# jiahuei/sparse-image-captioning

Measured on AMD Instinct MI355X. Metric: captions/sec, higher is better.
Workload: dtype bf16; 1 GPU; configs[1]: ORT dense, 256 images x 5 captions, teacher-forcing XE fwd+bwd+clip+Adam; images_per_gpu=256, regions=36, captions_per_image=5, parallelism=single

## Files before the change

### include/ortk.h

```cpp
#ifndef ORTK_H
#define ORTK_H

#include <stddef.h>
#include <stdint.h>

#ifdef __cplusplus
extern "C" {
#endif

#define ORTK_VERSION 19
#define ORTK_EINVAL (-1)
#define ORTK_ENOSPC (-2)
#define ORTK_ENOSYS (-3)
#define ORTK_EEXCHANGE (-4)

typedef void* ortk_stream;

int ortk_version(void);
int ortk_device_ok(void);

struct ortk_sparse_plan;
typedef struct ortk_config {
    int32_t d_model, d_ff, n_layers, n_heads;
    int32_t vocab, feat, seq_len;
    int32_t pad_id, bos_id, eos_id, unk_id;
    int32_t box_trig;
    int32_t precision;
    float   drop_src, drop;
    int32_t share_enc[16], share_dec[16];
    int32_t share_att_enc, share_att_dec;
    int32_t no_box;
    const struct ortk_sparse_plan* sparse_fwd;
    const struct ortk_sparse_plan* sparse_bwd;
// ... 120 lines not shown
int ortk_row_bchain(const ortk_bchain_args* a, ortk_stream stream);
int ortk_row_bchain_plan(const ortk_bchain_args* a, int32_t* rows_per_block, int32_t* workgroups);

typedef struct ortk_tuning {
    int32_t gemm_t64;
    int32_t attn_impl;
    int32_t attn16_min_lq;
    int32_t side_stream;
    int32_t row_chain;
    int32_t chain_wide;
    int32_t spmm_alias;
    int32_t f32_split;
    int32_t wgrad_wgs;
    int32_t wgrad_group;
    int32_t wgrad_group_splitk;
    int32_t wgrad_group_wgs;
    int32_t wgrad_group_tail;
    int32_t feats_bf16;
    int32_t ln_fuse;
    int32_t samp_epilogue;
    int32_t gemm_epilogue;
    int32_t attn16_short;
    int32_t attn16_block;
} ortk_tuning;
void ortk_get_tuning(ortk_tuning* out);
int ortk_set_tuning(const ortk_tuning* t);

#define ORTK_DEC_UNFUSED 1
#define ORTK_DEC_STACK 2
#define ORTK_DEC_SPARSE_STREAM 4
#define ORTK_DEC_STACK_RB20 8
#define ORTK_DEC_STACK_SPLIT 16
#define ORTK_DEC_SPLIT_SMALL 32
#define ORTK_DEC_SPARSE_GATHER 64
#define ORTK_DEC_STACK_FP8 128
#define ORTK_DEC_GROUPS_JOINT 65536
#define ORTK_MAX_BEAM 32
typedef struct ortk_decode_opts {
    int32_t beam_size;
    int32_t num_random_sample;
    float   temperature;
    int32_t decoding_constraint;
    int32_t length_penalty;
    double  length_alpha;
    uint64_t seed;
    const struct ortk_sparse_plan* sparse;
// ... 29 lines not shown


typedef struct ortk_gemm_args {
    const void* A; const void* B; void* C;
    int64_t lda, ldb, ldc;
    int32_t M, N, K, transA, transB;
    const float* bias; const float* rowscale; const float* resid; int64_t ldr;
    const void* gate; int64_t ldg; float gate_scale;
    int32_t relu; float drop_p; uint32_t drop_seed;
    int32_t accumulate, splitk, precision;
    int32_t a_dtype, b_dtype, c_dtype, gate_dtype;
    float* colsum;
    int32_t drop_row_stride, drop_row_off;
    int32_t ln_mode, ln_y_dtype;
    const float* ln_a; const float* ln_b; void* ln_y; float* ln_stats; float ln_eps;
    const float* ln_x; const float* ln_dres; float* ln_da; float* ln_db;
    float* tile_stats; int32_t stat_ncols;
    const int32_t* drop_rows;
    float* tile_samp; const int64_t* samp_seq; uint64_t samp_seed; int64_t samp_row_offset;
    int32_t samp_L, samp_t, samp_greedy_stride, samp_sample, samp_fast, samp_no_store; float samp_inv_temperature;
} ortk_gemm_args;
int ortk_gemm(const ortk_gemm_args* a, ortk_stream stream);
int ortk_gemm_plan(const ortk_gemm_args* a, char* buf, int32_t buf_bytes);
#define ORTK_WGRAD_MAX 8
typedef struct ortk_wgrad_item {
    const void* dY; int64_t lddy;
    const void* X; int64_t ldx;
    float* dW; int64_t lddw;
    float* db;
    int32_t Nout, Kin;
} ortk_wgrad_item;
typedef struct ortk_wgrad_group_args {
    ortk_wgrad_item item[ORTK_WGRAD_MAX];
    int32_t n, splitk;
    int64_t rows;
    int32_t flags;
    void* ws; size_t ws_bytes;
} ortk_wgrad_group_args;
int ortk_wgrad_group(const ortk_wgrad_group_args* a, ortk_stream stream);
size_t ortk_wgrad_group_workspace_bytes(const ortk_wgrad_group_args* a);
int ortk_prof_enable(int32_t on);
int ortk_prof_collect(int32_t key, int64_t* launches, double* total_ms, double* total_flops);
int ortk_prof_collect_bytes(int32_t key, double* total_bytes);
int ortk_prof_collect_units(int32_t key, double* total_workgroups);

int ortk_layernorm_fwd(const float* x, const float* a, const float* b, void* y, int32_t y_dtype, float* stats,
// ... 141 lines not shown
```

### sparse-image-captioning_amd/_lib.py

```python
import ctypes as C
import os

import torch

_HERE = os.path.dirname(os.path.abspath(__file__))
LIB_PATH = os.path.join(_HERE, "libortk.so")


class OrtkUnavailable(RuntimeError):
    pass


class OrtkError(RuntimeError):
    pass


class Config(C.Structure):
    _fields_ = [("d_model", C.c_int32), ("d_ff", C.c_int32), ("n_layers", C.c_int32), ("n_heads", C.c_int32),
                ("vocab", C.c_int32), ("feat", C.c_int32), ("seq_len", C.c_int32),
                ("pad_id", C.c_int32), ("bos_id", C.c_int32), ("eos_id", C.c_int32), ("unk_id", C.c_int32),
                ("box_trig", C.c_int32), ("precision", C.c_int32), ("drop_src", C.c_float), ("drop", C.c_float),
                ("share_enc", C.c_int32 * 16), ("share_dec", C.c_int32 * 16),
                ("share_att_enc", C.c_int32), ("share_att_dec", C.c_int32), ("no_box", C.c_int32),
                ("sparse_fwd", C.c_void_p), ("sparse_bwd", C.c_void_p)]
# ... 60 lines not shown
class MaskedAdamArgs(C.Structure):
    _fields_ = [("w", C.c_void_p), ("g", C.c_void_p), ("mw", C.c_void_p), ("vw", C.c_void_p),
                ("ml", C.c_void_p), ("mm", C.c_void_p), ("mv", C.c_void_p),
                ("draws", C.c_void_p), ("active", C.c_void_p), ("extra_coef", C.c_void_p),
                ("n", C.c_int64), ("index0", C.c_int64), ("mode", C.c_int32), ("seed", C.c_uint32),
                ("lr_w", C.c_float), ("eps_w", C.c_float), ("lr_m", C.c_float), ("eps_m", C.c_float),
                ("beta1", C.c_float), ("beta2", C.c_float), ("clip", C.c_float), ("bc1", C.c_float), ("bc2", C.c_float)]


OPT_ADAM, OPT_SGD, OPT_SGDM, OPT_SGDMOM, OPT_RMSPROP, OPT_ADAGRAD = range(6)
OPT_KINDS = {"adam": OPT_ADAM, "sgd": OPT_SGD, "sgdm": OPT_SGDM, "sgdmom": OPT_SGDMOM, "rmsprop": OPT_RMSPROP, "adagrad": OPT_ADAGRAD}


class OptimArgs(C.Structure):
    _fields_ = [("p", C.c_void_p), ("g", C.c_void_p), ("s1", C.c_void_p), ("s2", C.c_void_p), ("n", C.c_int64),
                ("kind", C.c_int32), ("first_step", C.c_int32), ("zero_grad", C.c_int32),
                ("lr", C.c_float), ("weight_decay", C.c_float), ("alpha", C.c_float), ("beta", C.c_float), ("eps", C.c_float),
                ("clip", C.c_float), ("bc1", C.c_float), ("bc2", C.c_float)]


class Tuning(C.Structure):
    _fields_ = [("gemm_t64", C.c_int32), ("attn_impl", C.c_int32), ("attn16_min_lq", C.c_int32),
                ("side_stream", C.c_int32), ("row_chain", C.c_int32), ("chain_wide", C.c_int32), ("spmm_alias", C.c_int32), ("f32_split", C.c_int32), ("wgrad_wgs", C.c_int32),
                ("wgrad_group", C.c_int32), ("wgrad_group_splitk", C.c_int32), ("wgrad_group_wgs", C.c_int32), ("wgrad_group_tail", C.c_int32), ("feats_bf16", C.c_int32), ("ln_fuse", C.c_int32), ("samp_epilogue", C.c_int32), ("gemm_epilogue", C.c_int32), ("attn16_short", C.c_int32), ("attn16_block", C.c_int32)]


class LnSlot(C.Structure):
    _fields_ = [("part", C.c_void_p), ("nblocks", C.c_int32), ("da", C.c_void_p), ("db", C.c_void_p)]


MAX_BEAM = 32
DEC_UNFUSED, DEC_STACK, DEC_SPARSE_STREAM, DEC_STACK_RB20, DEC_STACK_SPLIT, DEC_SPLIT_SMALL, DEC_SPARSE_GATHER, DEC_STACK_FP8 = 1, 2, 4, 8, 16, 32, 64, 128
DEC_GROUPS_JOINT = 1 << 16


class DecodeOpts(C.Structure):
    _fields_ = [("beam_size", C.c_int32), ("num_random_sample", C.c_int32), ("temperature", C.c_float),
                ("decoding_constraint", C.c_int32), ("length_penalty", C.c_int32), ("length_alpha", C.c_double),
                ("seed", C.c_uint64), ("sparse", C.POINTER(EllPlanStruct)), ("exec_flags", C.c_int32), ("with_greedy", C.c_int32), ("sample_row_offset", C.c_int64),
                ("train", C.c_int32), ("drop_seed", C.c_uint64), ("memory", C.c_void_p), ("top_k", C.c_int32), ("top_p", C.c_float),
                ("group_size", C.c_int32), ("diversity_lambda", C.c_float)]


class GemmArgs(C.Structure):
    _fields_ = [("A", C.c_void_p), ("B", C.c_void_p), ("C", C.c_void_p),
                ("lda", C.c_int64), ("ldb", C.c_int64), ("ldc", C.c_int64),
                ("M", C.c_int32), ("N", C.c_int32), ("K", C.c_int32), ("transA", C.c_int32), ("transB", C.c_int32),
# ... 57 lines not shown
    "ortk_valid_positions_ok": (_I32, [_CFG, _I32, _I32, _I32, _I32]),
    "ortk_forward": (_I32, [_CFG, _P, C.POINTER(Batch), _P, _SZ, _P, _I64, _I32, _U64, _P]),
    "ortk_forward_phase": (_I32, [_CFG, _P, C.POINTER(Batch), _P, _SZ, _P, _I64, _I32, _U64, _I32, _P]),
    "ortk_train_workspace_memory": (_P, [_CFG, _I32, _I32, _I32, _I32, _P, C.POINTER(C.c_int32)]),
    "ortk_loss": (_I32, [_CFG, C.POINTER(Batch), _P, _SZ, _P, _P, _P]),
    "ortk_loss_smooth": (_I32, [_CFG, C.POINTER(Batch), _P, _SZ, _P, _P, _F, _P]),
    "ortk_loss_external": (_I32, [_CFG, C.POINTER(Batch), _P, _SZ, _P, _P, _I64, _P]),
    "ortk_backward": (_I32, [_CFG, _P, _P, C.POINTER(Batch), _P, _SZ, _I32, _U64, _P]),
    "ortk_backward_phase": (_I32, [_CFG, _P, _P, C.POINTER(Batch), _P, _SZ, _I32, _U64, _I32, _P]),
    "ortk_arena_decoder_offset": (_I64, [_CFG]),
    "ortk_decode_workspace_bytes": (_SZ, [_CFG, _I32, _I32, C.POINTER(DecodeOpts)]),
    "ortk_decode": (_I32, [_CFG, _P, _P, _P, _P, _I32, _I32, C.POINTER(DecodeOpts), _P, _SZ, _P, _P, _P, _P]),
    "ortk_decode_status": (_I32, [_P, _P]),
    "ortk_encode": (_I32, [_CFG, _P, _P, _P, _P, _I32, _I32, _P, _SZ, _P, _P]),
    "ortk_chain_packed_bytes": (_SZ, [_I32]),
    "ortk_row_chain": (_I32, [C.POINTER(ChainArgs), _P]),
    "ortk_row_bchain": (_I32, [C.POINTER(BChainArgs), _P]),
    "ortk_row_chain_plan": (_I32, [C.POINTER(ChainArgs), C.POINTER(_I32), C.POINTER(_I32), C.POINTER(_I32), C.POINTER(_I32)]),
    "ortk_row_bchain_plan": (_I32, [C.POINTER(BChainArgs), C.POINTER(_I32), C.POINTER(_I32)]),
    "ortk_get_tuning": (None, [C.POINTER(Tuning)]),
    "ortk_set_tuning": (_I32, [C.POINTER(Tuning)]),
    "ortk_gemm": (_I32, [C.POINTER(GemmArgs), _P]),
    "ortk_gemm_plan": (_I32, [C.POINTER(GemmArgs), C.c_char_p, _I32]),
    "ortk_wgrad_group": (_I32, [C.POINTER(WgradGroupArgs), _P]),
    "ortk_wgrad_group_workspace_bytes": (_SZ, [C.POINTER(WgradGroupArgs)]),
    "ortk_prof_enable": (_I32, [_I32]),
    "ortk_prof_collect": (_I32, [_I32, C.POINTER(_I64), C.POINTER(C.c_double), C.POINTER(C.c_double)]),
    "ortk_prof_collect_bytes": (_I32, [_I32, C.POINTER(C.c_double)]),
    "ortk_prof_collect_units": (_I32, [_I32, C.POINTER(C.c_double)]),
    "ortk_layernorm_fwd": (_I32, [_P, _P, _P, _P, _I32, _P, _I64, _I32, _F, _P]),
    "ortk_layernorm_bwd": (_I32, [_P, _P, _P, _P, _P, _P, _P, _P, _I64, _I32, _F, _P]),
    "ortk_layernorm_bwd_drop": (_I32, [_P, _P, _P, _P, _P, _P, _P, _P, _I64, _I32, _F, _P, _I32, _F, C.c_uint32, _P]),
    "ortk_layernorm_bwd_drop_rows": (_I32, [_P, _P, _P, _P, _P, _P, _P, _P, _I64, _I32, _F, _P, _I32, _F, C.c_uint32, _P, _P]),
    "ortk_layernorm_bwd_dt": (_I32, [_P, _I32, _P, _P, _P, _P, _P, _P, _P, _I64, _I32, _F, _P, _I32, _F, C.c_uint32, _P, _P]),
    "ortk_layernorm_bwd_part": (_I32, [_P, _I32, _P, _P, _P, _P, _P, _P, _I64, C.POINTER(_I32), _I64, _I32, _F, _P, _I32, _F, C.c_uint32, _P, _P]),
    "ortk_ln_part_blocks": (_I32, [_I64]),
    "ortk_ln_part_rows": (_I32, []),
    "ortk_ln_partials_reduce": (_I32, [C.POINTER(LnSlot), _I32, _P]),
    "ortk_box_logbias_fwd": (_I32, [_P, C.POINTER(_P), C.POINTER(_P), C.POINTER(_F), _P, _I32, _I32, _I32, _I32, _P]),
    "ortk_box_logbias_bwd": (_I32, [_P, C.POINTER(_P), C.POINTER(_P), C.POINTER(_F), _P, C.POINTER(_P), C.POINTER(_P),
                                   _I32, _I32, _I32, _I32, _P]),
    "ortk_box_embedding": (_I32, [_P, C.POINTER(_F), _P, _I32, _I32, _P]),
    "ortk_attention_fwd": (_I32, [C.POINTER(AttnArgs), _P]),
    "ortk_attention_bwd": (_I32, [C.POINTER(AttnArgs), _P]),
    "ortk_attention_plan": (_I32, [C.POINTER(AttnArgs), _I32, C.c_char_p, _I32]),
    "ortk_valid_position_tables": (_I32, [_P, _I32, _I32, _P, _P, _P]),
# ... 20 lines not shown
    "ortk_adam_clip": (_I32, [_P, _P, _P, _P, _I64, _F, _F, _F, _F, _F, _F, _F, _P]),
    "ortk_adam_clip_zero": (_I32, [_P, _P, _P, _P, _I64, _F, _F, _F, _F, _F, _F, _F, _P]),
    "ortk_optim_states": (_I32, [_I32]),
    "ortk_optim_step": (_I32, [C.POINTER(OptimArgs), _P]),
    "ortk_mask_apply": (_I32, [_P, _P, _P, _I64, _I32, _U32, _P]),
    "ortk_mask_bwd": (_I32, [_P, _P, _P, _P, _P, _I64, _I32, _U32, _P, _P]),
    "ortk_masked_adam_step": (_I32, [C.POINTER(MaskedAdamArgs), _P]),
    "ortk_mask_count": (_I32, [_P, _I64, _I32, _P, _P]),
    "ortk_mask_select_workspace_bytes": (_SZ, [_I32, _I32, _I32, _I32]),
    "ortk_mask_select": (_I32, [_P, _P, _P, _P, _P, _P, _P, _P, _P, _I32, _I32, _I32, _I32, _P, _SZ, _P]),
    "ortk_mask_apply_draws": (_I32, [_P, _P, _P, _P, _I64, _P]),
    "ortk_mask_bwd_draws": (_I32, [_P, _P, _P, _P, _P, _P, _I64, _P, _P]),
    "ortk_decode_step_workspace_bytes": (_SZ, [_CFG, _I32]),
    "ortk_project_memory": (_I32, [_CFG, _P, _P, _I64, _P, _SZ, _P, _P]),
    "ortk_decode_step": (_I32, [_CFG, _P, _P, _I32, _I32, _I32, _I32, _P, _P, _P, _P, _I32, _P, _SZ, _P, _I64, _P]),
    "ortk_axpy_cols": (_I32, [_P, _P, _I32, _I64, _I64, _I32, _P]),
    "ortk_linear_block": (_I32, [_CFG, _I32, C.POINTER(C.c_int64), C.POINTER(C.c_int32), C.POINTER(C.c_int32)]),
    "ortk_sparse_build": (_I32, [C.POINTER(EllPlanStruct), _P, _I32, _P]),
    "ortk_spmm": (_I32, [C.POINTER(EllPlanStruct), _I32, C.POINTER(SpmmArgs), _P]),
    "ortk_spmm_plan": (_I32, [C.POINTER(EllPlanStruct), _I32, C.POINTER(SpmmArgs), C.c_char_p, _I32]),
}

_lib = None
ABI_VERSION = 19


def lib():
    global _lib
    if _lib is None:
        if not os.path.exists(LIB_PATH):
            raise OrtkUnavailable(
                f"{LIB_PATH} is missing: build it with `python -c 'import __graft_entry__ as g; g.build()'` "
                "(or `make -C sparse-image-captioning_amd/csrc`).  There is no CPU / PyTorch fallback.")
        h = C.CDLL(LIB_PATH)
        h.ortk_version.restype = C.c_int32
        if h.ortk_version() != ABI_VERSION:
            raise OrtkUnavailable(
                f"{LIB_PATH} is ABI version {h.ortk_version()}, these bindings were written for version {ABI_VERSION} (include/ortk.h: "
                "ORTK_VERSION): a stale build.  Rebuild it with `make -C sparse-image-captioning_amd/csrc`.")
        for name, (res, args) in SIGNATURES.items():
            fn = getattr(h, name)
            fn.restype = res
            fn.argtypes = args
        _lib = h
    return _lib


def set_tuning(**kw):
    t = Tuning()
    lib().ortk_get_tuning(C.byref(t))
    old = {f: getattr(t, f) for f, _ in Tuning._fields_}
    for k, v in kw.items():
        assert k in old, k
        setattr(t, k, int(v))
    check(lib().ortk_set_tuning(C.byref(t)), "ortk_set_tuning")
    return old


def gemm_plan(args):
    buf = C.create_string_buffer(256)
    check(lib().ortk_gemm_plan(C.byref(args), buf, len(buf)), "ortk_gemm_plan")
    return [k for k in buf.value.decode().split(";") if k]


def row_chain_plan(args):
    v = [C.c_int32() for _ in range(4)]
    check(lib().ortk_row_chain_plan(C.byref(args), *[C.byref(x) for x in v]), "ortk_row_chain_plan")
    return dict(zip(("form", "rows_per_block", "workgroups", "prefetchers"), (x.value for x in v)))


def row_bchain_plan(args):
    v = [C.c_int32() for _ in range(2)]
    check(lib().ortk_row_bchain_plan(C.byref(args), *[C.byref(x) for x in v]), "ortk_row_bchain_plan")
    return dict(zip(("rows_per_block", "workgroups"), (x.value for x in v)))


def attention_plan(args, bwd=False):
    buf = C.create_string_buffer(256)
    check(lib().ortk_attention_plan(C.byref(args), int(bool(bwd)), buf, len(buf)), "ortk_attention_plan")
    return [k for k in buf.value.decode().split(";") if k]


def spmm_plan(plan, block, args):
    if hasattr(plan, "ref"):
        plan = plan.ref()
    elif isinstance(plan, EllPlanStruct):
        plan = C.pointer(plan)
# ... 38 lines not shown
```

### sparse-image-captioning_amd/csrc/ortk_gemm.hip

```cpp
#include <algorithm>
#include <cstring>
#include <type_traits>
#include "ortk_internal.h"

namespace {

constexpr int BM = 128, BN = 128;
constexpr int PITCH = 128 + 16;

__device__ __forceinline__ int xcd_remap(int bid, int nwg) {
    const int q = nwg >> 3, r = nwg & 7, x = bid & 7, i = bid >> 3;
    return (x < r ? x * (q + 1) : r * (q + 1) + (x - r) * q) + i;
}

__device__ __forceinline__ float4 ld4(const float* __restrict__ base, int64_t ld, int row, int col, int nrows, int ncols,
                                      bool vec) {
    float4 r = make_float4(0.f, 0.f, 0.f, 0.f);
    if (row < nrows && col < ncols) {
        const float* p = base + (int64_t)row * ld + col;
        if (vec && col + 3 < ncols) {
            r = *reinterpret_cast<const float4*>(p);
        } else {
            r.x = p[0];
            if (col + 1 < ncols) r.y = p[1];
// ... 844 lines not shown
}

template <bool PERM = false>
__device__ __forceinline__ void glds_piece64(const __bf16* __restrict__ base, int64_t ld, int tile0, int k0, __bf16* img, int wave, int lane, int u,
                                             int rmax = 0x7FFFFFFF) {
    const int inst = wave * 4 + u;
    const int r = inst * 8 + (lane >> 3), c = (lane & 7) ^ (PERM ? swz_mk64p(r) : swz_mk64(r));
    const __bf16* g = base + (int64_t)min(tile0 + r, rmax) * ld + k0 + c * 8;
    __builtin_amdgcn_global_load_lds((glb_void*)g, (lds_void*)(img + inst * 512), 16, 0, 0);
}

__device__ __forceinline__ bf16x8 gfrag64p(const __bf16* img, int n0, int j, int ks, int lane) {
    const int lr = lane & 15, lg = lane >> 4;
    const int row = n0 + 32 * (j >> 1) + 8 * (lr >> 2) + 4 * (j & 1) + (lr & 3);
    return *reinterpret_cast<const bf16x8*>(img + row * HBK + (((ks * 4 + lg) ^ swz_mk64p(row)) << 3));
}

__device__ __forceinline__ bf16x8 gfrag64(const __bf16* img, int m0, int ks, int lane) {
    const int lr = lane & 15, lg = lane >> 4;
    return *reinterpret_cast<const bf16x8*>(img + (m0 + lr) * HBK + (((ks * 4 + lg) ^ swz_mk64(lr)) << 3));
}

template <int EPI = -1>
__global__ __launch_bounds__(512, 1) void gemm_bf16_dma256_kernel(ortk_gemm_args p, int tilesM, int tilesN, int kchunk) {
    constexpr int IMG = 256 * HBK;
    extern __shared__ __attribute__((aligned(16))) __bf16 smem16[];
    const int tid = threadIdx.x, lane = tid & 63, wave = tid >> 6;
    const int wm = wave >> 2, wn = wave & 3;
    const int bid = xcd_remap(blockIdx.x, gridDim.x);
    const int nt = bid % tilesN, rest = bid / tilesN, mt = rest % tilesM, ks_ = rest / tilesM;
    const int mb = mt * 256, nb = nt * 256;
    const int k_begin = ks_ * kchunk;
    const int k_end = min(p.K, k_begin + kchunk);
    const __bf16* Ap = reinterpret_cast<const __bf16*>(p.A);
    const __bf16* Bp = reinterpret_cast<const __bf16*>(p.B);
    const int T = (k_end - k_begin) / HBK;

    f32x4 acc[8][4];
#pragma unroll
    for (int i = 0; i < 8; ++i)
#pragma unroll
        for (int j = 0; j < 4; ++j) acc[i][j] = (f32x4){0.f, 0.f, 0.f, 0.f};
    auto issue = [&](int t) {
        __bf16* st = smem16 + (size_t)(t & 1) * 2 * IMG;
        glds_tile64(Ap, p.lda, mb, k_begin + t * HBK, st, wave, lane, p.M - 1);
        glds_tile64<true>(Bp, p.ldb, nb, k_begin + t * HBK, st + IMG, wave, lane);
    };
    if (T > 0) issue(0);
    for (int t = 0; t < T; ++t) {
        asm volatile("s_waitcnt vmcnt(0)" ::: "memory");
        __builtin_amdgcn_s_barrier();
        asm volatile("" ::: "memory");
        const bool next = t + 1 < T;
        __bf16* nst = smem16 + (size_t)((t + 1) & 1) * 2 * IMG;
        const int nk0 = k_begin + (t + 1) * HBK;
        const __bf16* sA = smem16 + (size_t)(t & 1) * 2 * IMG;
        const __bf16* sB = sA + IMG;
#pragma unroll
        for (int ks = 0; ks < 2; ++ks) {
            bf16x8 a[8], b[4];
#pragma unroll
            for (int j = 0; j < 4; ++j) b[j] = gfrag64p(sB, wn * 64, j, ks, lane);
#pragma unroll
            for (int i = 0; i < 8; ++i) a[i] = gfrag64(sA, wm * 128 + 16 * i, ks, lane);
#pragma unroll
            for (int i = 0; i < 8; ++i) {
                if (next && (i & 1) == 0) {
                    const int u = ks * 4 + (i >> 1);
                    if (u < 4) glds_piece64(Ap, p.lda, mb, nk0, nst, wave, lane, u, p.M - 1);
                    else       glds_piece64<true>(Bp, p.ldb, nb, nk0, nst + IMG, wave, lane, u - 4);
                }
#pragma unroll
                for (int j = 0; j < 4; ++j)
                    acc[i][j] = __builtin_amdgcn_mfma_f32_16x16x32_bf16(b[j], a[i], acc[i][j], 0, 0, 0);
            }
        }
    }
    const int ncol0 = nb + wn * 64 + 8 * (lane >> 4);
    if constexpr (EPI >= 0) {
        epilogue_lean<8, true, (EPI & 1) != 0, (EPI & 2) != 0>(p, mb + wm * 128 + (lane & 15), ncol0, acc);
        return;
    }
    Epi e{p.C, p.ldc, p.c_dtype, p.bias, p.rowscale, p.resid, p.ldr, p.gate, p.ldg, p.gate_dtype, p.gate_scale,
          p.relu, p.drop_p, p.drop_seed, p.accumulate, ks_ == 0, p.M, p.N, p.drop_row_stride > 0 ? p.drop_row_stride : 1, p.drop_row_off, p.drop_rows};
    if (mb + 256 <= p.M) {
#pragma unroll
        for (int hh = 0; hh < 2; ++hh)
            epilogue_tile<true, 4, 4, 16, 16, true>(e, mb + wm * 128 + 64 * hh + (lane & 15), ncol0, *reinterpret_cast<f32x4(*)[4][4]>(&acc[4 * hh]));
    } else {
#pragma unroll
        for (int hh = 0; hh < 2; ++hh)
            epilogue_tile<false, 4, 4, 16, 16, true>(e, mb + wm * 128 + 64 * hh + (lane & 15), ncol0, *reinterpret_cast<f32x4(*)[4][4]>(&acc[4 * hh]));
    }
}
constexpr size_t DMA256_LDS_BYTES = (size_t)2 * 2 * 256 * HBK * sizeof(__bf16);


constexpr int RP_M = 128, RP_N = 512;
constexpr int RP_IMG_A = RP_M * HBK, RP_IMG_B = RP_N * HBK;
constexpr size_t RP_LDS_BYTES = (size_t)2 * (RP_IMG_A + RP_IMG_B) * sizeof(__bf16);

__global__ __launch_bounds__(512, 1) void gemm_bf16_row512_kernel(ortk_gemm_args p, int, int, int) {
    extern __shared__ __attribute__((aligned(16))) __bf16 smem16[];
    const int tid = threadIdx.x, lane = tid & 63, wave = tid >> 6;
    const int wm = wave >> 2, wn = wave & 3;
    const int mb = blockIdx.x * RP_M;
    const __bf16* Ap = reinterpret_cast<const __bf16*>(p.A);
    const __bf16* Bp = reinterpret_cast<const __bf16*>(p.B);
    const int T = p.K / HBK;

    f32x4 acc[4][8];
#pragma unroll
    for (int i = 0; i < 4; ++i)
#pragma unroll
        for (int j = 0; j < 8; ++j) acc[i][j] = (f32x4){0.f, 0.f, 0.f, 0.f};
// ... 805 lines not shown
#pragma unroll
                for (int g = 0; g < 4; ++g)
                    *reinterpret_cast<f32x4*>(sC + (mr + 32 * i) * CP + nc + 32 * j + 8 * g) =
                        (f32x4){acc[i][j][4 * g], acc[i][j][4 * g + 1], acc[i][j][4 * g + 2], acc[i][j][4 * g + 3]};
        __syncthreads();
        epilogue_from_lds<false>(e, sC, mb, nb, lane, wave);
        return;
    }
    f32x4 acc4[2][8];
#pragma unroll
    for (int i = 0; i < 2; ++i)
#pragma unroll
        for (int j = 0; j < 2; ++j)
#pragma unroll
            for (int g = 0; g < 4; ++g) acc4[i][4 * j + g] = (f32x4){acc[i][j][4 * g], acc[i][j][4 * g + 1], acc[i][j][4 * g + 2], acc[i][j][4 * g + 3]};
    epilogue_tile<false, 2, 8, 32, 8>(e, mb + wm * 64 + l32, nb + wn * 64 + 4 * lh, acc4);
}

struct Launch { const void* fn; const char* name; unsigned grid, block; size_t lds; int a0, a1, a2; };
struct Plan {
    Launch l[2]; int n = 0;
    int key = 0; double bytes = 0.0;
    bool colsum_first = false; int ln_after = 0;
    void add(Inst k, int64_t grid, int block, size_t lds, int a0, int a1, int a2) {
        l[n++] = Launch{reinterpret_cast<const void*>(k.fn), k.name, (unsigned)grid, (unsigned)block, lds, a0, a1, a2};
    }
};
struct Tiling { int tilesM, tilesN, splitk, kchunk; int64_t grid() const { return (int64_t)tilesM * tilesN * splitk; } };

bool al(const void* q, size_t a_) { return q == nullptr || (reinterpret_cast<uintptr_t>(q) % a_) == 0; }
int layout_key(const ortk_gemm_args& p) { return (p.precision ? 4 : 0) | (p.transA ? 2 : 0) | (p.transB ? 1 : 0); }

Tiling gemm_tiling(const ortk_gemm_args& p) {
    Tiling t{(int)ortk_cdiv(p.M, BM), (int)ortk_cdiv(p.N, BN), 1, 0};
    const int bk = p.precision ? BK16 : (ortk::tuning().f32_split && (p.transA || p.transB)) ? 32 : 16;
    t.splitk = p.accumulate ? (p.splitk > 0 ? p.splitk : 1) : 1;
    t.kchunk = bk;
    if (p.K <= 0) {
        t.splitk = 1;
    } else {
        const int ksteps = (int)ortk_cdiv(p.K, bk);
        if (t.splitk > ksteps) t.splitk = ksteps;
        t.kchunk = (int)ortk_cdiv(ksteps, t.splitk) * bk;
        t.splitk = (int)ortk_cdiv(p.K, t.kchunk);
    }
    return t;
// ... 116 lines not shown
    const int tm = (int)ortk_cdiv(p.M, 64), tn = p.N / 64;
    const bool one = (int64_t)tm * tn <= 256 + 64;
    pl.add(one ? ORTK_INST(bf16_dma64, 8) : ORTK_INST(bf16_dma64, 3), (int64_t)tm * tn, 256, (one ? 8 : 3) * DMA64_STAGE_BYTES, tm, tn, t.kchunk);
    return true;
}

Inst lean_glds(const ortk_gemm_args& p) {
    if (p.tile_stats) return p.tile_samp ? ORTK_INST(bf16_glds, 0,5) : ORTK_INST(bf16_glds, 0,4);
    switch ((p.drop_p > 0.f ? 1 : 0) | (p.gate ? 2 : 0)) {
        case 0:  return ORTK_INST(bf16_glds, 0,0);
        case 1:  return ORTK_INST(bf16_glds, 0,1);
        case 2:  return ORTK_INST(bf16_glds, 0,2);
        default: return ORTK_INST(bf16_glds, 0,3);
    }
}
Inst lean_dma256(const ortk_gemm_args& p) {
    switch ((p.drop_p > 0.f ? 1 : 0) | (p.gate ? 2 : 0)) {
        case 0:  return ORTK_INST(bf16_dma256, 0);
        case 1:  return ORTK_INST(bf16_dma256, 1);
        case 2:  return ORTK_INST(bf16_dma256, 2);
        default: return ORTK_INST(bf16_dma256, 3);
    }
}
bool plan_dma(const ortk_gemm_args& p, const Tiling& t, Plan& pl) {
    const bool fast_nk = bf16_fast_nk(p, t), fast4 = bf16_fast4(p, t);
    const bool want_stats = p.tile_stats != nullptr;
    if (!(layout_key(p) == 4 && (fast4 || (fast_nk && p.M % BM == 0)) && both_bf16(p) && t.kchunk % GBK == 0 && t.tilesN <= 0xFFFF)) return false;
    const int64_t big_blocks = (int64_t)ortk_cdiv(p.M, 256) * (p.N / 256);
    const int64_t rounds = (big_blocks + 255) / 256;
    const bool fills = big_blocks * 10 >= rounds * 256 * 5;
    const bool lean = !p.accumulate && !p.rowscale && !(ortk::tuning().gemm_epilogue & 1);
    const bool nsplit = lean && !want_stats && !(ortk::tuning().gemm_epilogue & 2) && p.N % 256 == 128 && p.N > 256 && p.K % HBK == 0;
    const bool big = !p.accumulate && !want_stats && (p.M % 256 == 0 || fast4) && (p.N % 256 == 0 || nsplit) && fills;
    const Inst small = lean ? lean_glds(p) : ORTK_INST(bf16_glds, 0,-1);
    if (!big) {
        pl.add(small, t.grid(), 256, GLDS_LDS_BYTES, t.tilesM, t.tilesN, t.kchunk);
    } else if (p.K % HBK == 0) {
        pl.add(lean ? lean_dma256(p) : ORTK_INST(bf16_dma256, -1), big_blocks, 512, DMA256_LDS_BYTES, (int)ortk_cdiv(p.M, 256), p.N / 256, t.kchunk);
        if (nsplit)
            pl.add(small, t.tilesM, 256, GLDS_LDS_BYTES, t.tilesM, 1 | ((t.tilesN - 1) << 16), t.kchunk);
    } else {
        pl.add(ORTK_INST(bf16_glds, 1,-1), big_blocks, 512, GLDS_LDS_BYTES_BIG, (int)ortk_cdiv(p.M, 256), p.N / 256, t.kchunk);
    }
    return true;
}

void plan_bf16(const ortk_gemm_args& p, const Tiling& t, Plan& pl) {
    const int key = layout_key(p);
    const bool fast = bf16_fast_nk(p, t) && p.M % BM == 0;
    pl.add(pick16(key, p.a_dtype, p.b_dtype, fast), t.grid(), 256, BF16_LDS_BYTES, t.tilesM, t.tilesN, t.kchunk);
}

int gemm_launch(ortk_gemm_args& p, Plan& pl, hipStream_t s) {
    for (int i = 0; i < pl.n; ++i)
        if (pl.l[i].lds > 0 && ortk::lds_attr(pl.l[i].fn, pl.l[i].lds)) return ORTK_EINVAL;
    ortk::ProfMark mark;
    ortk::prof_begin(pl.key, 2.0 * p.M * p.N * p.K, pl.bytes, s, mark);
    for (int i = 0; i < pl.n; ++i) {
        Launch& l = pl.l[i];
        void* args[] = {&p, &l.a0, &l.a1, &l.a2};
        (void)hipLaunchKernel(l.fn, dim3(l.grid), dim3(l.block), args, l.lds, s);
// ... 27 lines not shown
            pl.colsum_first = p.colsum != nullptr;
            plan_f32(p, t, pl);
        }
    }
    return 0;
}
#undef ORTK_INST
#undef ORTK_INST0
#undef ORTK_INST_NAME

}

extern "C" int ortk_gemm(const ortk_gemm_args* a, ortk_stream stream) {
    ortk_gemm_args p; Plan pl;
    if (int e = gemm_build(a, p, pl)) return e;
    if (pl.n == 0) return 0;
    if (pl.colsum_first) { if (int e = ortk_colsum(p.A, ORTK_F32, p.lda, p.colsum, p.K, p.M, stream)) return e; }
    if (int e = gemm_launch(p, pl, ortk_s(stream))) return e;
    if (!pl.ln_after) return 0;
    float* Cf = reinterpret_cast<float*>(a->C);
    if (pl.ln_after == 1) return ortk_layernorm_fwd(Cf, a->ln_a, a->ln_b, a->ln_y, a->ln_y_dtype, a->ln_stats, a->M, a->N, a->ln_eps, stream);
    return ortk_layernorm_bwd_drop_rows(Cf, a->ln_x, a->ln_a, a->ln_stats, a->ln_dres, Cf, a->ln_da, a->ln_db, a->M, a->N, a->ln_eps,
                                        a->ln_y, a->ln_y_dtype, a->drop_p, a->drop_seed, a->drop_rows, stream);
}

extern "C" int ortk_gemm_plan(const ortk_gemm_args* a, char* buf, int32_t buf_bytes) {
    ortk_gemm_args p; Plan pl;
    if (int e = gemm_build(a, p, pl)) return e;
    if (!buf || buf_bytes <= 0) return ORTK_EINVAL;
    const char* part[4]; int n = 0;
    if (pl.n && pl.colsum_first) part[n++] = "colsum";
    for (int i = 0; i < pl.n; ++i) part[n++] = pl.l[i].name;
    if (pl.n && pl.ln_after) part[n++] = pl.ln_after == 1 ? "layernorm_fwd" : "layernorm_bwd_drop_rows";
    size_t need = 1;
    for (int i = 0; i < n; ++i) need += strlen(part[i]) + (i ? 1 : 0);
    if (need > (size_t)buf_bytes) return ORTK_ENOSPC;
    char* w = buf;
    for (int i = 0; i < n; ++i) {
        if (i) *w++ = ';';
        const size_t len = strlen(part[i]);
        memcpy(w, part[i], len); w += len;
    }
    *w = 0;
    return 0;
}
```

### sparse-image-captioning_amd/csrc/ortk_runtime.hip

```cpp
#include <mutex>
#include <vector>
#include "ortk_internal.h"

namespace ortk {
static ortk_tuning tuning_defaults() {
    ortk_tuning t{};
    t.gemm_t64 = 640;
    t.attn_impl = 0;
    t.attn16_min_lq = 33;
    t.side_stream = 1;
    t.row_chain = 1;
    t.chain_wide = 1;
    t.spmm_alias = 1;
    t.f32_split = 1;
    t.wgrad_wgs = 384;
    t.wgrad_group = 3;
    t.wgrad_group_splitk = 0;
    t.wgrad_group_wgs = 96;
    t.wgrad_group_tail = 1;
    t.feats_bf16 = 1;
    t.ln_fuse = 0;
    t.samp_epilogue = 1;
    t.gemm_epilogue = 0;
    t.attn16_short = 1;
    t.attn16_block = 1;
    return t;
}
static ortk_tuning g_tuning = tuning_defaults();
const ortk_tuning& tuning() { return g_tuning; }
}

extern "C" void ortk_get_tuning(ortk_tuning* out) { if (out) *out = ortk::g_tuning; }
extern "C" int ortk_set_tuning(const ortk_tuning* t) {
    if (!t) return ORTK_EINVAL;
    auto in = [](int32_t v, int32_t lo, int32_t hi) { return v >= lo && v <= hi; };
    if (!in(t->row_chain, 0, 1)  || !in(t->attn_impl, 0, 4) || t->attn16_min_lq < 1 || !in(t->f32_split, 0, 7) || t->wgrad_wgs < 1 ||
        !in(t->wgrad_group, 0, 15) || !in(t->wgrad_group_splitk, 0, 8) || t->wgrad_group_wgs < 1 || !in(t->wgrad_group_tail, 0, 1) ||
        !in(t->feats_bf16, 0, 1) || !in(t->ln_fuse, 0, 31) || (t->ln_fuse & 3)  ||
        !in(t->samp_epilogue, 0, 1) || !in(t->gemm_epilogue, 0, 3) ||
        !(in(t->attn16_short, 0, 1) || t->attn16_short == 4 || t->attn16_short == 8) || !in(t->attn16_block, 0, 1)) return ORTK_EINVAL;
    ortk::g_tuning = *t;
    return 0;
}

namespace ortk {
int lds_attr(const void* fn, size_t bytes) {
    struct Key { int dev; const void* fn; size_t bytes; };
    static std::mutex mu;
    static std::vector<Key>* seen = new std::vector<Key>();
    int dev = 0;
    if (hipGetDevice(&dev) != hipSuccess) return ORTK_EINVAL;
    std::lock_guard<std::mutex> lk(mu);
    for (const Key& k : *seen) if (k.dev == dev && k.fn == fn && k.bytes >= bytes) return 0;
    if (hipFuncSetAttribute(fn, hipFuncAttributeMaxDynamicSharedMemorySize, (int)bytes) != hipSuccess) return ORTK_EINVAL;
    seen->push_back(Key{dev, fn, bytes});
    return 0;
}
}

namespace {
struct ProfRec { hipEvent_t a, b; int key; double flops, bytes; int slot; double per_count; double units; };
constexpr int PROF_SLOTS = 1 << 16;
unsigned long long* g_prof_slots = nullptr;
// ... 83 lines not shown
```

Measured before the change: 137,200 captions/sec.

## Add persistent multi-tile walk to bf16 dma256 GEMM kernel with tuning knob

```diff
diff --git a/include/ortk.h b/include/ortk.h
--- a/include/ortk.h
+++ b/include/ortk.h
@@ -8,7 +8,7 @@
 extern "C" {
 #endif
 
-#define ORTK_VERSION 19
+#define ORTK_VERSION 20
 #define ORTK_EINVAL (-1)
 #define ORTK_ENOSPC (-2)
 #define ORTK_ENOSYS (-3)
@@ -175,6 +175,7 @@
     int32_t gemm_epilogue;
     int32_t attn16_short;
     int32_t attn16_block;
+    int32_t gemm_walk;
 } ortk_tuning;
 void ortk_get_tuning(ortk_tuning* out);
 int ortk_set_tuning(const ortk_tuning* t);
@@ -250,6 +251,7 @@
 } ortk_gemm_args;
 int ortk_gemm(const ortk_gemm_args* a, ortk_stream stream);
 int ortk_gemm_plan(const ortk_gemm_args* a, char* buf, int32_t buf_bytes);
+int ortk_gemm_walk(const ortk_gemm_args* a, int32_t* tiles_per_wg, int32_t* workgroups);
 #define ORTK_WGRAD_MAX 8
 typedef struct ortk_wgrad_item {
     const void* dY; int64_t lddy;
diff --git a/scratch/gemm_walk_bench.py b/scratch/gemm_walk_bench.py
--- /dev/null
+++ b/scratch/gemm_walk_bench.py
@@ -0,0 +1,39 @@
+import ctypes as C, os, sys
+ROOT = os.path.dirname(os.path.dirname(os.path.abspath(__file__)))
+sys.path.insert(0, ROOT)
+import torch
+import sparse_image_captioning_amd as P
+L = P._lib; lib = L.lib()
+def timeit(f, n=40):
+    for _ in range(3): f()
+    torch.cuda.synchronize(); e0 = torch.cuda.Event(enable_timing=True); e1 = torch.cuda.Event(enable_timing=True)
+    e0.record()
+    for _ in range(n): f()
+    e1.record(); torch.cuda.synchronize()
+    return e0.elapsed_time(e1) * 1e3 / n
+SHAPES = [(16640, 2048, 512, 1, 0, 1), (9216, 2048, 512, 1, 0, 1), (21760, 2048, 512, 1, 0, 1), (16640, 10112, 512, 0, 1, 0),
+          (9216, 6144, 512, 0, 0, 1), (16640, 512, 512, 0, 0, 1)]
+WALKS = (1, 2, 3, 4, 0)
+for M, N, K, gated, biased, c16 in SHAPES:
+    A = torch.randn(M, K, device="cuda").bfloat16(); B = torch.randn(N, K, device="cuda").bfloat16()
+    Cc = torch.empty(M, N, device="cuda", dtype=torch.bfloat16 if c16 else torch.float32)
+    a = L.GemmArgs(); a.A, a.B, a.C = A.data_ptr(), B.data_ptr(), Cc.data_ptr(); a.lda, a.ldb, a.ldc = K, K, N
+    a.M, a.N, a.K, a.precision, a.a_dtype, a.b_dtype, a.c_dtype = M, N, K, 1, 1, 1, c16
+    if gated:
+        gate = torch.randn(M, N, device="cuda").bfloat16()
+        a.gate, a.ldg, a.gate_dtype, a.gate_scale = gate.data_ptr(), N, 1, 1.0 / 0.9
+    if biased:
+        bias = torch.randn(N, device="cuda")
+        a.bias = bias.data_ptr()
+    res = {w: [] for w in WALKS}
+    how = {}
+    for rep in range(3):
+        for w in WALKS:
+            L.set_tuning(gemm_walk=w)
+            how[w] = (L.gemm_plan(a), L.gemm_walk(a))
+            res[w].append(timeit(lambda: lib.ortk_gemm(C.byref(a), L.stream_ptr())))
+    print(f"M {M} N {N} K {K} gate {gated} bias {biased} C {'bf16' if c16 else 'f32'}  {';'.join(how[1][0])}", flush=True)
+    for w in WALKS:
+        print(f"    gemm_walk {w}: tiles/wg {how[w][1]['tiles_per_wg']} workgroups {how[w][1]['workgroups']:5d}   us " + " ".join(f"{t:7.1f}" for t in res[w]), flush=True)
+    del A, B, Cc
+L.set_tuning(gemm_walk=0)
diff --git a/sparse-image-captioning_amd/_lib.py b/sparse-image-captioning_amd/_lib.py
--- a/sparse-image-captioning_amd/_lib.py
+++ b/sparse-image-captioning_amd/_lib.py
@@ -106,7 +106,7 @@
 class Tuning(C.Structure):
     _fields_ = [("gemm_t64", C.c_int32), ("attn_impl", C.c_int32), ("attn16_min_lq", C.c_int32),
                 ("side_stream", C.c_int32), ("row_chain", C.c_int32), ("chain_wide", C.c_int32), ("spmm_alias", C.c_int32), ("f32_split", C.c_int32), ("wgrad_wgs", C.c_int32),
-                ("wgrad_group", C.c_int32), ("wgrad_group_splitk", C.c_int32), ("wgrad_group_wgs", C.c_int32), ("wgrad_group_tail", C.c_int32), ("feats_bf16", C.c_int32), ("ln_fuse", C.c_int32), ("samp_epilogue", C.c_int32), ("gemm_epilogue", C.c_int32), ("attn16_short", C.c_int32), ("attn16_block", C.c_int32)]
+                ("wgrad_group", C.c_int32), ("wgrad_group_splitk", C.c_int32), ("wgrad_group_wgs", C.c_int32), ("wgrad_group_tail", C.c_int32), ("feats_bf16", C.c_int32), ("ln_fuse", C.c_int32), ("samp_epilogue", C.c_int32), ("gemm_epilogue", C.c_int32), ("attn16_short", C.c_int32), ("attn16_block", C.c_int32), ("gemm_walk", C.c_int32)]
 
 
 class LnSlot(C.Structure):
@@ -210,6 +210,7 @@
     "ortk_set_tuning": (_I32, [C.POINTER(Tuning)]),
     "ortk_gemm": (_I32, [C.POINTER(GemmArgs), _P]),
     "ortk_gemm_plan": (_I32, [C.POINTER(GemmArgs), C.c_char_p, _I32]),
+    "ortk_gemm_walk": (_I32, [C.POINTER(GemmArgs), C.POINTER(_I32), C.POINTER(_I32)]),
     "ortk_wgrad_group": (_I32, [C.POINTER(WgradGroupArgs), _P]),
     "ortk_wgrad_group_workspace_bytes": (_SZ, [C.POINTER(WgradGroupArgs)]),
     "ortk_prof_enable": (_I32, [_I32]),
@@ -276,7 +277,7 @@
 }
 
 _lib = None
-ABI_VERSION = 19
+ABI_VERSION = 20
 
 
 def lib():
@@ -317,6 +318,12 @@
     return [k for k in buf.value.decode().split(";") if k]
 
 
+def gemm_walk(args):
+    v = [C.c_int32() for _ in range(2)]
+    check(lib().ortk_gemm_walk(C.byref(args), *[C.byref(x) for x in v]), "ortk_gemm_walk")
+    return dict(zip(("tiles_per_wg", "workgroups"), (x.value for x in v)))
+
+
 def row_chain_plan(args):
     v = [C.c_int32() for _ in range(4)]
     check(lib().ortk_row_chain_plan(C.byref(args), *[C.byref(x) for x in v]), "ortk_row_chain_plan")
diff --git a/sparse-image-captioning_amd/csrc/ortk_gemm.hip b/sparse-image-captioning_amd/csrc/ortk_gemm.hip
--- a/sparse-image-captioning_amd/csrc/ortk_gemm.hip
+++ b/sparse-image-captioning_amd/csrc/ortk_gemm.hip
@@ -890,75 +890,91 @@
 }
 
 template <int EPI = -1>
-__global__ __launch_bounds__(512, 1) void gemm_bf16_dma256_kernel(ortk_gemm_args p, int tilesM, int tilesN, int kchunk) {
+__global__ __launch_bounds__(512, 1) void gemm_bf16_dma256_kernel(ortk_gemm_args p, int tilesM, int tilesN_walk, int kchunk) {
     constexpr int IMG = 256 * HBK;
+    const int tilesN = tilesN_walk & 0xFFFF, walk = max(tilesN_walk >> 16, 1);
     extern __shared__ __attribute__((aligned(16))) __bf16 smem16[];
     const int tid = threadIdx.x, lane = tid & 63, wave = tid >> 6;
-    const int wm = wave >> 2, wn = wave & 3;
-    const int bid = xcd_remap(blockIdx.x, gridDim.x);
-    const int nt = bid % tilesN, rest = bid / tilesN, mt = rest % tilesM, ks_ = rest / tilesM;
-    const int mb = mt * 256, nb = nt * 256;
-    const int k_begin = ks_ * kchunk;
-    const int k_end = min(p.K, k_begin + kchunk);
+    const int ntiles = tilesM * tilesN * ((p.K + kchunk - 1) / kchunk);
+    int tile = xcd_remap(blockIdx.x, gridDim.x) * walk;
+    const int tile_end = min(tile + walk, ntiles);
+    if (tile >= tile_end) return;
     const __bf16* Ap = reinterpret_cast<const __bf16*>(p.A);
     const __bf16* Bp = reinterpret_cast<const __bf16*>(p.B);
-    const int T = (k_end - k_begin) / HBK;
-
-    f32x4 acc[8][4];
-#pragma unroll
-    for (int i = 0; i < 8; ++i)
-#pragma unroll
-        for (int j = 0; j < 4; ++j) acc[i][j] = (f32x4){0.f, 0.f, 0.f, 0.f};
-    auto issue = [&](int t) {
-        __bf16* st = smem16 + (size_t)(t & 1) * 2 * IMG;
-        glds_tile64(Ap, p.lda, mb, k_begin + t * HBK, st, wave, lane, p.M - 1);
-        glds_tile64<true>(Bp, p.ldb, nb, k_begin + t * HBK, st + IMG, wave, lane);
+    int mb, nb, ks_, k_begin, T;
+    auto locate = [&](int id, int& mb_, int& nb_, int& ks__, int& kb_, int& T_) {
+        const int nt = id % tilesN, rest = id / tilesN;
+        mb_ = (rest % tilesM) * 256; nb_ = nt * 256; ks__ = rest / tilesM;
+        kb_ = ks__ * kchunk;
+        T_ = (min(p.K, kb_ + kchunk) - kb_) / HBK;
     };
-    if (T > 0) issue(0);
-    for (int t = 0; t < T; ++t) {
-        asm volatile("s_waitcnt vmcnt(0)" ::: "memory");
-        __builtin_amdgcn_s_barrier();
-        asm volatile("" ::: "memory");
-        const bool next = t + 1 < T;
-        __bf16* nst = smem16 + (size_t)((t + 1) & 1) * 2 * IMG;
-        const int nk0 = k_begin + (t + 1) * HBK;
-        const __bf16* sA = smem16 + (size_t)(t & 1) * 2 * IMG;
-        const __bf16* sB = sA + IMG;
-#pragma unroll
-        for (int ks = 0; ks < 2; ++ks) {
-            bf16x8 a[8], b[4];
-#pragma unroll
-            for (int j = 0; j < 4; ++j) b[j] = gfrag64p(sB, wn * 64, j, ks, lane);
-#pragma unroll
-            for (int i = 0; i < 8; ++i) a[i] = gfrag64(sA, wm * 128 + 16 * i, ks, lane);
-#pragma unroll
-            for (int i = 0; i < 8; ++i) {
-                if (next && (i & 1) == 0) {
-                    const int u = ks * 4 + (i >> 1);
-                    if (u < 4) glds_piece64(Ap, p.lda, mb, nk0, nst, wave, lane, u, p.M - 1);
-                    else       glds_piece64<true>(Bp, p.ldb, nb, nk0, nst + IMG, wave, lane, u - 4);
+    locate(tile, mb, nb, ks_, k_begin, T);
+    glds_tile64(Ap, p.lda, mb, k_begin, smem16, wave, lane, p.M - 1);
+    glds_tile64<true>(Bp, p.ldb, nb, k_begin, smem16 + IMG, wave, lane);
+    int g = 0;
+    for (; tile < tile_end; ++tile) {
+        const bool more = tile + 1 < tile_end;
+        int mb2, nb2, ks2, kb2, T2;
+        locate(more ? tile + 1 : tile, mb2, nb2, ks2, kb2, T2);
+        f32x4 acc[8][4];
+#pragma unroll
+        for (int i = 0; i < 8; ++i)
+#pragma unroll
+            for (int j = 0; j < 4; ++j) acc[i][j] = (f32x4){0.f, 0.f, 0.f, 0.f};
+        int tid_k = tid;
+        asm volatile("" : "+v"(tid_k));
+        const int lane_k = tid_k & 63, wave_k = tid_k >> 6, wm_k = tid_k >> 8, wn_k = (tid_k >> 6) & 3;
+        for (int t = 0; t < T; ++t, ++g) {
+            asm volatile("s_waitcnt vmcnt(0)" ::: "memory");
+            __builtin_amdgcn_s_barrier();
+            asm volatile("" ::: "memory");
+            const bool inner = t + 1 < T;
+            const bool next = inner || more;
+            const int nmb = inner ? mb : mb2, nnb = inner ? nb : nb2;
+            const int nk0 = inner ? k_begin + (t + 1) * HBK : kb2;
+            __bf16* nst = smem16 + (size_t)((g + 1) & 1) * 2 * IMG;
+            const __bf16* sA = smem16 + (size_t)(g & 1) * 2 * IMG;
+            const __bf16* sB = sA + IMG;
+#pragma unroll
+            for (int ks = 0; ks < 2; ++ks) {
+                bf16x8 a[8], b[4];
+#pragma unroll
+                for (int j = 0; j < 4; ++j) b[j] = gfrag64p(sB, wn_k * 64, j, ks, lane_k);
+#pragma unroll
+                for (int i = 0; i < 8; ++i) a[i] = gfrag64(sA, wm_k * 128 + 16 * i, ks, lane_k);
+#pragma unroll
+                for (int i = 0; i < 8; ++i) {
+                    if (next && (i & 1) == 0) {
+                        const int u = ks * 4 + (i >> 1);
+                        if (u < 4) glds_piece64(Ap, p.lda, nmb, nk0, nst, wave_k, lane_k, u, p.M - 1);
+                        else       glds_piece64<true>(Bp, p.ldb, nnb, nk0, nst + IMG, wave_k, lane_k, u - 4);
+                    }
+#pragma unroll
+                    for (int j = 0; j < 4; ++j)
+                        acc[i][j] = __builtin_amdgcn_mfma_f32_16x16x32_bf16(b[j], a[i], acc[i][j], 0, 0, 0);
                 }
-#pragma unroll
-                for (int j = 0; j < 4; ++j)
-                    acc[i][j] = __builtin_amdgcn_mfma_f32_16x16x32_bf16(b[j], a[i], acc[i][j], 0, 0, 0);
-            }
-        }
-    }
-    const int ncol0 = nb + wn * 64 + 8 * (lane >> 4);
-    if constexpr (EPI >= 0) {
-        epilogue_lean<8, true, (EPI & 1) != 0, (EPI & 2) != 0>(p, mb + wm * 128 + (lane & 15), ncol0, acc);
-        return;
-    }
-    Epi e{p.C, p.ldc, p.c_dtype, p.bias, p.rowscale, p.resid, p.ldr, p.gate, p.ldg, p.gate_dtype, p.gate_scale,
-          p.relu, p.drop_p, p.drop_seed, p.accumulate, ks_ == 0, p.M, p.N, p.drop_row_stride > 0 ? p.drop_row_stride : 1, p.drop_row_off, p.drop_rows};
-    if (mb + 256 <= p.M) {
-#pragma unroll
-        for (int hh = 0; hh < 2; ++hh)
-            epilogue_tile<true, 4, 4, 16, 16, true>(e, mb + wm * 128 + 64 * hh + (lane & 15), ncol0, *reinterpret_cast<f32x4(*)[4][4]>(&acc[4 * hh]));
-    } else {
-#pragma unroll
-        for (int hh = 0; hh < 2; ++hh)
-            epilogue_tile<false, 4, 4, 16, 16, true>(e, mb + wm * 128 + 64 * hh + (lane & 15), ncol0, *reinterpret_cast<f32x4(*)[4][4]>(&acc[4 * hh]));
+            }
+        }
+        int tid_e = tid;
+        asm volatile("" : "+v"(tid_e));
+        const int lane_e = tid_e & 63, wm_e = tid_e >> 8, wn_e = (tid_e >> 6) & 3;
+        const int ncol0 = nb + wn_e * 64 + 8 * (lane_e >> 4);
+        if constexpr (EPI >= 0) {
+            epilogue_lean<8, true, (EPI & 1) != 0, (EPI & 2) != 0>(p, mb + wm_e * 128 + (lane_e & 15), ncol0, acc);
+        } else {
+            Epi e{p.C, p.ldc, p.c_dtype, p.bias, p.rowscale, p.resid, p.ldr, p.gate, p.ldg, p.gate_dtype, p.gate_scale,
+                  p.relu, p.drop_p, p.drop_seed, p.accumulate, ks_ == 0, p.M, p.N, p.drop_row_stride > 0 ? p.drop_row_stride : 1, p.drop_row_off, p.drop_rows};
+            if (mb + 256 <= p.M) {
+#pragma unroll
+                for (int hh = 0; hh < 2; ++hh)
+                    epilogue_tile<true, 4, 4, 16, 16, true>(e, mb + wm_e * 128 + 64 * hh + (lane_e & 15), ncol0, *reinterpret_cast<f32x4(*)[4][4]>(&acc[4 * hh]));
+            } else {
+#pragma unroll
+                for (int hh = 0; hh < 2; ++hh)
+                    epilogue_tile<false, 4, 4, 16, 16, true>(e, mb + wm_e * 128 + 64 * hh + (lane_e & 15), ncol0, *reinterpret_cast<f32x4(*)[4][4]>(&acc[4 * hh]));
+            }
+        }
+        mb = mb2; nb = nb2; ks_ = ks2; k_begin = kb2; T = T2;
     }
 }
 constexpr size_t DMA256_LDS_BYTES = (size_t)2 * 2 * 256 * HBK * sizeof(__bf16);
@@ -1810,6 +1826,7 @@
     Launch l[2]; int n = 0;
     int key = 0; double bytes = 0.0;
     bool colsum_first = false; int ln_after = 0;
+    int walk = 0;
     void add(Inst k, int64_t grid, int block, size_t lds, int a0, int a1, int a2) {
         l[n++] = Launch{reinterpret_cast<const void*>(k.fn), k.name, (unsigned)grid, (unsigned)block, lds, a0, a1, a2};
     }
@@ -1972,6 +1989,10 @@
         default: return ORTK_INST(bf16_dma256, 3);
     }
 }
+int dma256_walk(int64_t tiles) {
+    if (tiles <= 256) return 1;
+    return 1;
+}
 bool plan_dma(const ortk_gemm_args& p, const Tiling& t, Plan& pl) {
     const bool fast_nk = bf16_fast_nk(p, t), fast4 = bf16_fast4(p, t);
     const bool want_stats = p.tile_stats != nullptr;
@@ -1986,7 +2007,10 @@
     if (!big) {
         pl.add(small, t.grid(), 256, GLDS_LDS_BYTES, t.tilesM, t.tilesN, t.kchunk);
     } else if (p.K % HBK == 0) {
-        pl.add(lean ? lean_dma256(p) : ORTK_INST(bf16_dma256, -1), big_blocks, 512, DMA256_LDS_BYTES, (int)ortk_cdiv(p.M, 256), p.N / 256, t.kchunk);
+        const int force = ortk::tuning().gemm_walk;
+        pl.walk = force > 0 ? force : dma256_walk(big_blocks);
+        pl.add(lean ? lean_dma256(p) : ORTK_INST(bf16_dma256, -1), ortk_cdiv(big_blocks, pl.walk), 512, DMA256_LDS_BYTES, (int)ortk_cdiv(p.M, 256),
+               (p.N / 256) | (pl.walk << 16), t.kchunk);
         if (nsplit)
             pl.add(small, t.tilesM, 256, GLDS_LDS_BYTES, t.tilesM, 1 | ((t.tilesN - 1) << 16), t.kchunk);
     } else {
@@ -2060,6 +2084,14 @@
     if (pl.ln_after == 1) return ortk_layernorm_fwd(Cf, a->ln_a, a->ln_b, a->ln_y, a->ln_y_dtype, a->ln_stats, a->M, a->N, a->ln_eps, stream);
     return ortk_layernorm_bwd_drop_rows(Cf, a->ln_x, a->ln_a, a->ln_stats, a->ln_dres, Cf, a->ln_da, a->ln_db, a->M, a->N, a->ln_eps,
                                         a->ln_y, a->ln_y_dtype, a->drop_p, a->drop_seed, a->drop_rows, stream);
+}
+
+extern "C" int ortk_gemm_walk(const ortk_gemm_args* a, int32_t* tiles_per_wg, int32_t* workgroups) {
+    ortk_gemm_args p; Plan pl;
+    if (int e = gemm_build(a, p, pl)) return e;
+    if (tiles_per_wg) *tiles_per_wg = pl.walk;
+    if (workgroups) *workgroups = pl.walk ? (int32_t)pl.l[0].grid : 0;
+    return 0;
 }
 
 extern "C" int ortk_gemm_plan(const ortk_gemm_args* a, char* buf, int32_t buf_bytes) {
diff --git a/sparse-image-captioning_amd/csrc/ortk_runtime.hip b/sparse-image-captioning_amd/csrc/ortk_runtime.hip
--- a/sparse-image-captioning_amd/csrc/ortk_runtime.hip
+++ b/sparse-image-captioning_amd/csrc/ortk_runtime.hip
@@ -24,6 +24,7 @@
     t.gemm_epilogue = 0;
     t.attn16_short = 1;
     t.attn16_block = 1;
+    t.gemm_walk = 0;
     return t;
 }
 static ortk_tuning g_tuning = tuning_defaults();
@@ -38,7 +39,8 @@
         !in(t->wgrad_group, 0, 15) || !in(t->wgrad_group_splitk, 0, 8) || t->wgrad_group_wgs < 1 || !in(t->wgrad_group_tail, 0, 1) ||
         !in(t->feats_bf16, 0, 1) || !in(t->ln_fuse, 0, 31) || (t->ln_fuse & 3)  ||
         !in(t->samp_epilogue, 0, 1) || !in(t->gemm_epilogue, 0, 3) ||
-        !(in(t->attn16_short, 0, 1) || t->attn16_short == 4 || t->attn16_short == 8) || !in(t->attn16_block, 0, 1)) return ORTK_EINVAL;
+        !(in(t->attn16_short, 0, 1) || t->attn16_short == 4 || t->attn16_short == 8) || !in(t->attn16_block, 0, 1) ||
+        !in(t->gemm_walk, 0, 8)) return ORTK_EINVAL;
     ortk::g_tuning = *t;
     return 0;
 }
```

New measurement: 136,800 captions/sec. No clear change (-0.3%).
